# pennneutrinos/chroma

Hardware: AMD Instinct MI355X
Metric: photons/sec (propagate_hit) (higher is better)
Workload: dtype f32

## Files before the change

chroma_amd/csrc/chroma_hip.hip:

```cpp
#include <math.h>
#include <stdio.h>
#include <stdlib.h>
#include <string.h>
#include <algorithm>

#ifndef CHROMA_EXPERIMENTAL
#define CHROMA_EXPERIMENTAL 0
#endif
#ifndef CHROMA_HYBRID_RENDER
#define CHROMA_HYBRID_RENDER 1
#endif
#include "chroma_internal.h"
#include "propagate_device.h"

#include "kernel_propagate_fused.h"

#include "kernel_step_control.h"

#include "kernels_raycast_crosscheck.h"

#include "kernel_raycast_quad.h"

#include "kernel_raycast_pair.h"

// ... 123 lines not shown
        for (const Walk &w : WALKS)
            if (w.spill == b.kind) rays = std::max(rays, (size_t)ctx->waves[(int)w.cast] * w.rays_per_wave);
        HIP_TRY(hipSetDevice(ctx->device));
        HIP_TRY(ctx_malloc(ctx, (void **)b.buf, rays * b.depth * sizeof(uint2)));
    }
    return CHROMA_OK;
}

static unsigned cast_waves(const chroma_ctx *ctx, Cast cast, long long n)
{
    const long long per = WALKS[(int)cast].rays_per_wave;
    return (unsigned)std::min<long long>((n + per - 1) / per, ctx->waves[(int)cast]);
}

struct FusedLaunch { int first, nthreads; const uint32_t *in_q; uint32_t *out_q; int max_steps, use_weights, scatter_first; };
static int launch_propagate(const CallScope &scope, bool counting, chroma_geometry *geom, const PhotonView &pv, chroma_rng rng, const FusedLaunch &a)
{
    chroma_ctx *ctx = scope.ctx;
    const dim3 grid((unsigned)((a.nthreads + PROP_BLOCK - 1) / PROP_BLOCK)), block(PROP_BLOCK);
    with_bool(counting, [&](auto C) {
        hipLaunchKernelGGL((k_propagate<STACK_LDS, C>), grid, block, 0, ctx->stream, geom->view, pv, a.first, a.nthreads, a.in_q, a.out_q,
                           rng.seed, rng.photon_id_base, a.max_steps, a.use_weights, a.scatter_first, scope.state().d_counters);
    });
    HIP_TRY(hipGetLastError());
    return CHROMA_OK;
}

static int stats_read(const CallScope &scope, chroma_propagate_stats *stats)
{
    chroma_ctx *ctx = scope.ctx; CallState &cs = scope.state();
    DeviceCounters c;
    HIP_TRY(hipStreamSynchronize(ctx->stream));
    HIP_TRY(hipMemcpy(&c, cs.d_counters, sizeof c, hipMemcpyDeviceToHost));
    HIP_TRY(hipMemset(cs.d_counters, 0, sizeof c));
    stats->photon_steps += c.photon_steps;
    stats->nodes_visited += c.nodes_visited;
    stats->triangles_tested += c.triangles_tested;
    stats->stack_overflows += c.stack_overflows;
    stats->stack_spills += c.stack_spills;
    stats->packet_rays += c.packet_rays;
    stats->packet_nodes_visited += c.packet_nodes;
    stats->packet_triangles_tested += c.packet_tris;
    return CHROMA_OK;
}

enum { EV_STEP_BEGIN, EV_PACKET_BEGIN, EV_CAST_BEGIN, EV_CAST_END, EV_PHYSICS_END, EV_STEP_END, EV_PER_STEP };

struct chroma_tracks {
    struct Slab { float4 *rows; uint32_t count; };
    uint64_t nphotons = 0, nrows = 0;
    float4 *rows0 = nullptr;
    uint32_t *offsets = nullptr;
    std::vector<Slab> slabs;
};

static void tracks_release(chroma_ctx *ctx, chroma_tracks *tr)
{
    if (!tr) return;
    for (const chroma_tracks::Slab &s : tr->slabs) chroma_free(ctx, s.rows);
    chroma_free(ctx, tr->rows0);
    chroma_free(ctx, tr->offsets);
    delete tr;
}

namespace { struct PropagateCall; }
static int propagate_order(PropagateCall &call, uint32_t **d_order);

namespace {
struct PropagateCall {
    const CallScope &scope; CallState &cs;
    chroma_ctx *ctx; chroma_geometry *geom;
    CallPlan plan;
    PhotonView pv; chroma_rng rng; chroma_propagate_options opt;
    uint64_t nphotons; uint32_t ncopies;
    uint32_t *in_q, *out_q;
    float4 *work_in, *work_out;
    float4 *rays, *rays_next;
    float4 *final_rec;
    uint32_t final_epoch;
    HitsOut ho;
    bool finalize;
    chroma_propagate_stats acc;
    long long n_upper;
    bool finalized;
    chroma_tracks *tracks;

    hipEvent_t *events(int step) const { return opt.time_kernels ? cs.step_events.data() + EV_PER_STEP * step : nullptr; }

    int load_working()
    {
        const unsigned blocks = (unsigned)std::min<uint64_t>((nphotons + PHYS_BLOCK - 1) / PHYS_BLOCK, (uint64_t)ctx->physics_blocks);
        int rc = scope.clear_words(W_PACKET_USE, W_PACKET_END - W_PACKET_USE); if (rc) return rc;
        uint32_t *d_order = nullptr;
        rc = propagate_order(*this, &d_order); if (rc) return rc;
        hipLaunchKernelGGL(k_load_working, dim3(blocks), dim3(PHYS_BLOCK), 0, ctx->stream, geom->view, pv, in_q, work_in,
                           (uint64_t)nphotons, ncopies, (uint32_t)(nphotons / ncopies), plan.chain ? rays : nullptr,
                           plan.packet == 2 ? cs.d_words + W_PACKET_COHERENT : nullptr, (const uint32_t *)d_order, plan.cast == Cast::LITERAL ? 1 : 0);
        if (d_order) { chroma_free(ctx, d_order); acc.reordered += nphotons; }
#if CHROMA_EXPERIMENTAL
        if (plan.packet)
            hipLaunchKernelGGL(k_packet_decide, dim3(1), dim3(1), 0, ctx->stream, cs.d_words + W_PACKET_COHERENT, cs.d_words + W_PACKET_USE,
                               (uint64_t)nphotons, plan.packet);
#endif
        HIP_TRY(hipGetLastError());
        return CHROMA_OK;
    }

    void launch_step_begin(uint32_t first_n)
    {
        hipLaunchKernelGGL(k_step_begin, dim3(1), dim3(1), 0, ctx->stream, in_q, out_q, cs.d_step,
                           tracks ? 0u : opt.use_weights ? 0xFFFFFFFFu : (uint32_t)(PROP_BLOCK * 16 * 8), first_n);
    }

    void launch_physics(int scatter_first, int fixup)
    {
        StepState *st = cs.d_step;
        float4 *chained = plan.chain ? rays_next : nullptr;
        const bool plain = geom->view.plain_optics != 0;
        bool deal = false;
#if PHYS_DEAL
        deal = plain && !final_rec;
#endif
        const int pb = deal ? PHYS_DEAL_BLOCK : PHYS_BLOCK_OF(!plain);
        unsigned blocks = (unsigned)std::min<long long>((n_upper + pb - 1) / pb, std::max<long long>(1, (long long)ctx->physics_blocks * PHYS_BLOCK / pb));
        if (fixup == 1 && plain) blocks = std::max(std::min(blocks, 64u), blocks / 8);
        DeviceCounters *pc = plan.counting ? cs.d_counters : nullptr;
#if PHYS_DEAL
        if (deal) {
            hipLaunchKernelGGL(k_physics_deal, dim3(blocks), dim3(PHYS_DEAL_BLOCK), 0, ctx->stream, geom->view, pv, st, work_in, out_q, work_out,
                               cs.hit_triangle, cs.hit_distance, rng.seed, rng.photon_id_base, opt.use_weights, scatter_first,
                               cs.retry_list, fixup, pc, chained);
            return;
        }
#endif
        const int literal_rays = fixup == 2 ? 1 : 0;
        with_bool(!plain, [&](auto FULL) {
            hipLaunchKernelGGL((k_physics<FULL>), dim3(blocks), dim3(PHYS_BLOCK_OF(FULL)), 0, ctx->stream, geom->view, pv, st, work_in, out_q,
                               work_out, cs.hit_triangle, cs.hit_distance, rng.seed, rng.photon_id_base, opt.use_weights, scatter_first,
                               cs.retry_list, fixup, pc, chained, final_rec, final_epoch, literal_rays);
        });
    }

    int launch_split_step(int scatter_first, hipEvent_t *ev, uint32_t first_n, bool packet)
    {
        if (n_upper <= 0) return CHROMA_OK;
        StepState *st = cs.d_step;
        const Cast cast = plan.cast;
        const bool exact = cast == Cast::LITERAL || cast == Cast::LITERAL_LANE;
        const dim3 block(PROP_BLOCK);
        auto record = [&](int slot) { return ev ? hipEventRecord(ev[slot], ctx->stream) : hipSuccess; };
        const unsigned rblocks = (unsigned)std::min<long long>((n_upper + PROP_BLOCK - 1) / PROP_BLOCK, 8 * 256);
        auto retry = [&](auto C) {
            hipLaunchKernelGGL((k_raycast_retry<C>), dim3(rblocks), block, 0, ctx->stream, geom->view, rays, st, cs.hit_triangle,
                               cs.hit_distance, cs.retry_list, cs.d_counters);
        };
        launch_step_begin(first_n);
        HIP_TRY(record(EV_STEP_BEGIN));
        if (!plan.chain) {
            unsigned sblocks = (unsigned)std::min<long long>((n_upper + 255) / 256, (long long)ctx->physics_blocks * 4);
            hipLaunchKernelGGL(k_ray_setup, dim3(sblocks), dim3(256), 0, ctx->stream, geom->view, work_in, st, rays,
                               cs.hit_triangle, cs.hit_distance, cs.retry_list, &st->retry, cast == Cast::LITERAL ? 1 : 0);
        }
        HIP_TRY(record(EV_PACKET_BEGIN));
        const uint32_t *skip_quad = nullptr;
#if CHROMA_EXPERIMENTAL
        if (packet) {
            skip_quad = cs.d_words + W_PACKET_USE;
            const unsigned pwaves = (unsigned)std::min<long long>((n_upper + WAVE - 1) / WAVE, (long long)ctx->waves[(int)Cast::QUAD]);
            with_bool(plan.counting, [&](auto C) {
                hipLaunchKernelGGL((k_raycast_packet<C>), dim3(pwaves), block, 0, ctx->stream, geom->view, rays, st, cs.hit_triangle,
                                   cs.hit_distance, cs.retry_list, cs.d_counters, cs.d_words + W_PACKET_USE);
            });
        }
#else
        (void)packet;
#endif
        HIP_TRY(record(EV_CAST_BEGIN));
        const dim3 grid(cast_waves(ctx, cast, n_upper));
        const int chained = plan.chain ? 1 : 0;
        with_bool(plan.counting, [&](auto C) {
            switch (cast) {
            case Cast::PAIR:
                hipLaunchKernelGGL((k_raycast_pair<C>), grid, block, 0, ctx->stream, geom->view, rays, 0, st, cs.hit_triangle,
                                   cs.hit_distance, cs.retry_list, cs.coop_spill, cs.d_counters, ctx->coop_chunk);
                break;
            case Cast::QUAD:
                hipLaunchKernelGGL((k_raycast_quad<C>), grid, block, 0, ctx->stream, geom->view, rays, 0, st, cs.hit_triangle,
                                   cs.hit_distance, cs.retry_list, cs.coop_spill, cs.d_counters, ctx->coop_chunk, chained, skip_quad,
                                   ctx->claim_static);
                break;
            case Cast::COOP:
                hipLaunchKernelGGL((k_raycast_coop<C>), grid, block, 0, ctx->stream, geom->view, rays, 0, st, cs.hit_triangle,
                                   cs.hit_distance, cs.retry_list, cs.coop_spill, cs.d_counters, ctx->coop_chunk);
                break;
            case Cast::WIDE:
                hipLaunchKernelGGL((k_raycast_wide<C>), grid, block, 0, ctx->stream, geom->view, rays, 0, st, cs.hit_triangle,
                                   cs.hit_distance, cs.retry_list, cs.wide_spill, cs.d_counters, ctx->ray_chunk);
                break;
            case Cast::PERSISTENT:
                hipLaunchKernelGGL((k_raycast_persistent<C>), grid, block, 0, ctx->stream, geom->view, rays, 0, st, cs.hit_triangle,
                                   cs.hit_distance, cs.retry_list, cs.d_counters);
                break;
            case Cast::LITERAL:
                hipLaunchKernelGGL((k_raycast_literal<C>), grid, block, 0, ctx->stream, geom->view, rays, st, cs.hit_triangle,
                                   cs.hit_distance, cs.coop_spill, cs.d_counters, ctx->coop_chunk, chained, cs.retry_list,
                                   ctx->claim_static);
                retry(C);
                break;
            case Cast::LITERAL_LANE:
                hipLaunchKernelGGL((k_raycast_retry<C, true>), grid, block, 0, ctx->stream, geom->view, rays, st, cs.hit_triangle,
                                   cs.hit_distance, cs.retry_list, cs.d_counters);
                break;
            }
        });
        HIP_TRY(record(EV_CAST_END));
        launch_physics(scatter_first, exact ? 2 : 0);
        HIP_TRY(record(EV_PHYSICS_END));
        if (!exact) {
            with_bool(plan.counting, retry);
            launch_physics(scatter_first, 1);
        }
        HIP_TRY(record(EV_STEP_END));
        HIP_TRY(hipGetLastError());
        if (plan.chain) std::swap(rays, rays_next);
        return CHROMA_OK;
    }

    int launch_tail(int nsteps, int scatter_first, hipEvent_t *ev, uint32_t first_n, bool *done)
    {
        *done = false;
        const unsigned waves = cast_waves(ctx, Cast::COOP, n_upper);
        if ((long long)waves * 8 < n_upper) return CHROMA_OK;
        launch_step_begin(first_n);
        HitsOut beside; memset(&beside, 0, sizeof beside);
        uint32_t *words = nullptr;
        if (finalize) {
            beside = ho;
            words = cs.d_words;
            int rc = scope.clear_results(); if (rc) return rc;
            if (final_rec)
                hipLaunchKernelGGL(k_mark_tail, dim3(32), dim3(256), 0, ctx->stream, in_q, final_rec, photon_tail_stamp(final_epoch));
            HIP_TRY(hipEventRecord(cs.ev_fork, ctx->stream));
        }
        if (ev) HIP_TRY(hipEventRecord(ev[EV_STEP_BEGIN], ctx->stream));
        with_bool(plan.cast == Cast::LITERAL, [&](auto L) {
            with_bool(plan.counting, [&](auto C) {
                hipLaunchKernelGGL((k_tail_coop<C, L>), dim3(waves), dim3(PROP_BLOCK), 0, ctx->stream, geom->view, pv, cs.d_step, work_in,
                                   rng.seed, rng.photon_id_base, nsteps, opt.use_weights, scatter_first, cs.coop_spill, cs.d_counters, beside, words);
            });
        });
        if (ev) HIP_TRY(hipEventRecord(ev[EV_STEP_END], ctx->stream));
        if (finalize) {
            HIP_TRY(hipStreamWaitEvent(cs.aux_stream, cs.ev_fork, 0));
            launch_finalize(cs.aux_stream, photon_tail_stamp(final_epoch));
            HIP_TRY(hipEventRecord(cs.ev_join, cs.aux_stream));
            HIP_TRY(hipStreamWaitEvent(ctx->stream, cs.ev_join, 0));
            finalized = true;
        }
        HIP_TRY(hipGetLastError());
        *done = true;
        return CHROMA_OK;
    }

    void launch_finalize(hipStream_t stream, uint32_t tail_mark)
    {
        const unsigned blocks = (unsigned)((nphotons + COPY_ITEMS * 256 - 1) / (COPY_ITEMS * 256));
        hipLaunchKernelGGL(k_finalize_hits, dim3(blocks), dim3(256), 0, stream, geom->view, pv, (const float4 *)final_rec, final_epoch,
                           (uint64_t)nphotons, ho, cs.d_words, tail_mark);
    }

    int read_step_times(int steps, int tail_step)
    {
        for (int k = 0; k < steps; k++) {
            const hipEvent_t *ev = events(k);
            float ms = 0.f;
            HIP_TRY(hipEventElapsedTime(&ms, ev[EV_STEP_BEGIN], ev[EV_STEP_END]));
            acc.kernel_ms += ms;
            if (k == tail_step) continue;
            HIP_TRY(hipEventElapsedTime(&ms, ev[EV_CAST_BEGIN], ev[EV_CAST_END]));
            acc.raycast_ms += ms;
            acc.raycast_launches++;
            if (k == 0 && plan.packet) {
                HIP_TRY(hipEventElapsedTime(&ms, ev[EV_PACKET_BEGIN], ev[EV_CAST_BEGIN]));
                acc.packet_ms += ms;
                acc.packet_launches++;
            }
            HIP_TRY(hipEventElapsedTime(&ms, ev[EV_CAST_END], ev[EV_PHYSICS_END]));
            acc.physics_ms += ms;
            acc.physics_launches++;
        }
        return CHROMA_OK;
    }

    int run_device_steps()
    {
        const int max_steps = opt.max_steps;
        HIP_TRY(hipMemsetAsync(cs.d_step, 0, sizeof(StepState), ctx->stream));
        hipLaunchKernelGGL(k_set_word, dim3(1), dim3(1), 0, ctx->stream, in_q, 1u);
        hipLaunchKernelGGL(k_set_word, dim3(1), dim3(1), 0, ctx->stream, out_q, 1u);
        int rc = load_working(); if (rc) return rc;
        const int nev = opt.time_kernels ? EV_PER_STEP * max_steps : 0;
        while ((int)cs.step_events.size() < nev) { hipEvent_t e; HIP_TRY(hipEventCreate(&e)); cs.step_events.push_back(e); }
        const long long few = (long long)PROP_BLOCK * 16 * 8;
        int step = 0, next_check = 1, tail_step = -1;
        bool done = false;
        while (step < max_steps && !done) {
            const int scatter_first = step == 0 ? opt.scatter_first : 0;
            const uint32_t first_n = step == 0 ? (uint32_t)nphotons : 0u;
            if (plan.tail && n_upper < few) {
                rc = launch_tail(max_steps - step, scatter_first, events(step), first_n, &done); if (rc) return rc;
                if (done) { tail_step = step++; break; }
            }
            rc = launch_split_step(scatter_first, events(step), first_n, step == 0 && plan.packet != 0); if (rc) return rc;
            step++;
            std::swap(in_q, out_q);
            std::swap(work_in, work_out);
            if (step == next_check && step < max_steps) {
                rc = scope.read_survivors(in_q, &n_upper); if (rc) return rc;
                if (n_upper <= 0) done = true;
                next_check = (plan.tail_watch && n_upper < 16 * few) ? step + 1 : (step < 8) ? step * 2 : step + 8;
            }
        }
        if (!done) {
            unsigned blocks = (unsigned)std::min<long long>((n_upper + 255) / 256, 4096);
            hipLaunchKernelGGL(k_store_working, dim3(std::max(blocks, 1u)), dim3(256), 0, ctx->stream, geom->view, pv, in_q, work_in);
        }
        HIP_TRY(hipMemcpyAsync(cs.h_step, cs.d_step, sizeof(StepState), hipMemcpyDeviceToHost, ctx->stream));
        HIP_TRY(hipStreamSynchronize(ctx->stream));
        acc.launches += ((const StepState *)cs.h_step)->launches;
        return opt.time_kernels ? read_step_times(step, tail_step) : CHROMA_OK;
    }

    void store_working()
// ... 10 lines not shown
        hipLaunchKernelGGL(k_track_row0, dim3(tblocks), dim3(TRACK_BLOCK), 0, ctx->stream, pv, (uint64_t)nphotons, tr.rows0, tr.offsets,
                           (uint32_t)max_steps + 1u, max_steps >= 1 ? 2u : 1u);
        HIP_TRY(hipGetLastError());
        tr.nrows = nphotons;
        int step = 0;
        if (max_steps >= 1) {
            HIP_TRY(hipMemsetAsync(cs.d_step, 0, sizeof(StepState), ctx->stream));
            hipLaunchKernelGGL(k_set_word, dim3(1), dim3(1), 0, ctx->stream, in_q, 1u);
            hipLaunchKernelGGL(k_set_word, dim3(1), dim3(1), 0, ctx->stream, out_q, 1u);
            int rc = load_working(); if (rc) return rc;
            const int nev = opt.time_kernels ? EV_PER_STEP * max_steps : 0;
            while ((int)cs.step_events.size() < nev) { hipEvent_t e; HIP_TRY(hipEventCreate(&e)); cs.step_events.push_back(e); }
            rc = scope.read_survivors(in_q, &n_upper); if (rc) return rc;
            tr.nrows += nphotons - (uint64_t)n_upper;
            uint32_t *cursor = tr.offsets + nphotons + 1;
            while (step < max_steps && n_upper > 0) {
                const uint32_t n_in = (uint32_t)n_upper;
                chroma_tracks::Slab slab = {nullptr, n_in};
                if (step == 0) {
                    slab.rows = tr.slabs[0].rows;
                    tr.slabs.clear();
                    rc = CHROMA_OK;
                } else if (tr.nrows + n_in > max_rows)
                    rc = set_error(CHROMA_ERR_INVALID, "tracks: step %d would bring the call to %llu rows, more than the %llu of CHROMA_TRACKS_MAX_ROWS; %d steps were taken",
                                   step, (unsigned long long)(tr.nrows + n_in), (unsigned long long)max_rows, step);
                else
                    rc = chroma_malloc(ctx, (size_t)n_in * 4 * sizeof(float4), (void **)&slab.rows);
                if (rc) {
                    store_working();
                    hipStreamSynchronize(ctx->stream);
                    return rc;
                }
                tr.slabs.push_back(slab);
                HIP_TRY(hipMemsetAsync(cursor, 0, sizeof(uint32_t), ctx->stream));
                rc = launch_split_step(step == 0 ? opt.scatter_first : 0, events(step), step == 0 ? (uint32_t)nphotons : 0u, false);
                if (rc) return rc;
                const unsigned blocks = (unsigned)std::min<uint64_t>(((uint64_t)n_in + TRACK_BLOCK - 1) / TRACK_BLOCK, 4096);
                hipLaunchKernelGGL(k_track_step, dim3(blocks), dim3(TRACK_BLOCK), 0, ctx->stream, geom->view, pv, (const uint32_t *)in_q,
                                   (const uint32_t *)out_q, (const float4 *)work_out, slab.rows, n_in, cursor, tr.offsets, (uint32_t)step);
                HIP_TRY(hipGetLastError());
                tr.nrows += n_in;
                step++;
                std::swap(in_q, out_q);
                std::swap(work_in, work_out);
                rc = scope.read_survivors(in_q, &n_upper); if (rc) return rc;
            }
            if (n_upper > 0) store_working();
            HIP_TRY(hipMemcpyAsync(cs.h_step, cs.d_step, sizeof(StepState), hipMemcpyDeviceToHost, ctx->stream));
        }
        int rc = chroma_internal_exclusive_sum(ctx, tr.offsets, (uint32_t)nphotons + 1u); if (rc) return rc;
        HIP_TRY(hipStreamSynchronize(ctx->stream));
        uint32_t total = 0;
        HIP_TRY(hipMemcpy(&total, tr.offsets + nphotons, sizeof total, hipMemcpyDeviceToHost));
        if (total != tr.nrows)
            return set_error(CHROMA_ERR_INTERNAL, "tracks: %u rows recorded where the step counts give %llu", total, (unsigned long long)tr.nrows);
        if (max_steps >= 1) acc.launches += ((const StepState *)cs.h_step)->launches;
        return opt.time_kernels ? read_step_times(step, -1) : CHROMA_OK;
    }

    int run_fused()
    {
        hipLaunchKernelGGL(k_init_queue, dim3((unsigned)((nphotons + 255) / 256)), dim3(256), 0, ctx->stream, in_q,
                           (uint64_t)nphotons, ncopies, (uint32_t)(nphotons / ncopies));
        hipLaunchKernelGGL(k_set_word, dim3(1), dim3(1), 0, ctx->stream, out_q, 1u);
        HIP_TRY(hipGetLastError());
        const int max_steps = opt.max_steps;
        int scatter_first = opt.scatter_first;
        long long n = (long long)nphotons;
        int step = 0;
        while (step < max_steps) {
            const bool few = n < (long long)PROP_BLOCK * 16 * 8;
            int nsteps = (few || opt.use_weights) ? (max_steps - step) : 1;
            if (opt.time_kernels) HIP_TRY(hipEventRecord(cs.ev_start, ctx->stream));
            int rc = launch_propagate(scope, plan.counting, geom, pv, rng, {0, (int)n, in_q + 1, out_q, nsteps, opt.use_weights, scatter_first});
            if (rc) return rc;
            acc.launches++;
            if (opt.time_kernels) {
                HIP_TRY(hipEventRecord(cs.ev_stop, ctx->stream));
                HIP_TRY(hipEventSynchronize(cs.ev_stop));
                float ms = 0.f;
                HIP_TRY(hipEventElapsedTime(&ms, cs.ev_start, cs.ev_stop));
                acc.kernel_ms += ms;
            }
            step += nsteps;
            scatter_first = 0;
            if (step < max_steps) {
                std::swap(in_q, out_q);
                hipLaunchKernelGGL(k_set_word, dim3(1), dim3(1), 0, ctx->stream, out_q, 1u);
                rc = scope.read_survivors(in_q, &n); if (rc) return rc;
                if (n == 0) break;
            }
        }
        return CHROMA_OK;
    }

    int finish(chroma_hits_request *hr, chroma_propagate_stats *stats, int32_t *aborted)
    {
        int rc = CHROMA_OK;
        if (!finalize) {
            rc = scope.clear_words(W_ABORT); if (rc) return rc;
            const unsigned blocks = (unsigned)std::min<uint64_t>((nphotons + 255) / 256, 4096);
            hipLaunchKernelGGL(k_flags_or, dim3(blocks), dim3(256), 0, ctx->stream, pv.flags, (uint64_t)nphotons, CHROMA_NAN_ABORT,
                               cs.d_words + W_ABORT);
        } else if (!finalized) {
            rc = scope.clear_results(); if (rc) return rc;
            launch_finalize(ctx->stream, 0u);
        }
        HIP_TRY(hipGetLastError());
        rc = scope.read_results(); if (rc) return rc;
        if (hr) hr->nhits = scope.word(W_HIT_COUNT);
        if (aborted) *aborted = (scope.word(W_ABORT) & CHROMA_NAN_ABORT) ? 1 : 0;
        chroma_propagate_stats tmp; memset(&tmp, 0, sizeof tmp);
        chroma_propagate_stats *s = stats ? stats : &tmp;
        rc = stats_read(scope, s); if (rc) return rc;
        if (stats) {
            stats->launches += acc.launches;
            stats->kernel_ms += acc.kernel_ms;
            stats->raycast_ms += acc.raycast_ms;
            stats->raycast_launches += acc.raycast_launches;
            stats->physics_ms += acc.physics_ms;
            stats->physics_launches += acc.physics_launches;
            stats->packet_ms += acc.packet_ms;
            stats->packet_launches += acc.packet_launches;
            stats->reordered += acc.reordered;
        }
        if (s->stack_overflows) return set_error(CHROMA_ERR_STACK, "traversal stack overflowed for %llu rays", (unsigned long long)s->stack_overflows);
        return CHROMA_OK;
    }
};
}

int propagate_settings(const CallScope &scope)
{
    chroma_ctx *ctx = scope.ctx; CallState &cs = scope.state();
    hipDeviceProp_t prop;
    HIP_TRY(hipGetDeviceProperties(&prop, ctx->device));
    ctx->physics_blocks = prop.multiProcessorCount * 8;
    const char *walk = getenv("CHROMA_WALK");
    if (walk) cs.walk = CHROMA_WALK_QUAD;
    for (int w = 0; w < NWALKS; w++) {
        const Walk &row = WALKS[w];
        int per_cu = row.waves_per_cu;
        if (const char *e = getenv(row.waves_env)) per_cu = std::max(1, atoi(e));
        ctx->waves[(int)row.cast] = prop.multiProcessorCount * per_cu;
        if (walk && (!strcmp(walk, row.name) || (row.alias && !strcmp(walk, row.alias)))) cs.walk = w;
    }
#if CHROMA_EXPERIMENTAL
    if (const char *e = getenv("CHROMA_PACKET")) cs.packet_mode = !strcmp(e, "on") ? 1 : !strcmp(e, "auto") ? 2 : 0;
    if (const char *e = getenv("CHROMA_AUTOSORT")) cs.autosort_mode = !strcmp(e, "on") || !strcmp(e, "1") ? 1 : !strcmp(e, "off") || !strcmp(e, "0") ? 0 : 2;
#endif
    if (const char *e = getenv("CHROMA_RAY_CHUNK")) ctx->ray_chunk = std::max(64, atoi(e));
    if (const char *e = getenv("CHROMA_COOP_CHUNK")) ctx->coop_chunk = std::max(8, atoi(e));
    if (const char *e = getenv("CHROMA_CLAIM_STATIC")) { int big = 0, small = 0; if (sscanf(e, "%d:%d", &big, &small) < 2) small = big; ctx->claim_static = std::min(8, std::max(0, big)) | std::min(8, std::max(0, small)) << 4; }
    if (const char *e = getenv("CHROMA_TAIL"))
        cs.tail_mode = !strcmp(e, "fused") ? CHROMA_TAIL_FUSED : !strcmp(e, "split") ? CHROMA_TAIL_SPLIT : CHROMA_TAIL_COOP;
    return CHROMA_OK;
}

extern "C" {

int chroma_propagate_step(chroma_ctx *ctx, chroma_geometry *geom, int32_t first_photon, int32_t nthreads,
                          const uint32_t *d_input_queue, uint32_t *d_output_queue, chroma_rng rng,
                          const chroma_photon_arrays *photons, int32_t max_steps, int32_t use_weights,
                          int32_t scatter_first)
{
    if (!ctx || !geom) return set_error(CHROMA_ERR_INVALID, "bad argument");
    int rc = check_photons(photons, true);
    if (rc) return rc;
    if (first_photon < 0 || nthreads < 0) return set_error(CHROMA_ERR_INVALID, "negative photon range");
    if (nthreads == 0) return CHROMA_OK;
    if ((rc = check_stack(geom))) return rc;
    const CallScope scope(ctx);
    return launch_propagate(scope, scope.state().counting != 0, geom, to_view(photons), rng,
                            {first_photon, nthreads, d_input_queue, d_output_queue, max_steps, use_weights, scatter_first});
}

static int ensure_queues(const CallScope &scope, size_t n)
{
    chroma_ctx *ctx = scope.ctx; CallState &cs = scope.state();
    if (cs.queue_capacity >= n + 1) return CHROMA_OK;
    HIP_TRY(hipStreamSynchronize(ctx->stream));
    const auto buffers = queue_buffers(cs);
    for (const QueueBuffer &b : buffers) { if (*b.ptr) hipFree(*b.ptr); *b.ptr = nullptr; }
    cs.queue_capacity = 0;
    for (const QueueBuffer &b : buffers) HIP_TRY(ctx_malloc(ctx, b.ptr, (n + 1) * b.bytes));
    cs.queue_capacity = n + 1;
    return CHROMA_OK;
}

int chroma_distance_to_mesh(chroma_ctx *ctx, chroma_geometry *geom, int32_t nthreads, const float *d_origin,
                            const float *d_direction, float *d_distance, int32_t *d_triangle)
{
    return chroma_intersect_mesh(ctx, geom, nthreads, d_origin, d_direction, nullptr, d_distance, d_triangle);
}

int chroma_intersect_mesh(chroma_ctx *ctx, chroma_geometry *geom, int32_t nthreads, const float *d_origin,
                          const float *d_direction, const int32_t *d_last_hit, float *d_distance, int32_t *d_triangle)
{
    if (!ctx || !geom || !d_origin || !d_direction || !d_distance) return set_error(CHROMA_ERR_INVALID, "bad argument");
    if (nthreads <= 0) return CHROMA_OK;
    int rc = check_stack(geom); if (rc) return rc;
    const CallScope scope(ctx);
    CallState &cs = scope.state();
    CallPlan plan;
    rc = make_plan(cs, geom, -1, -1, -1, &plan); if (rc) return rc;
    if (!plan.isect_quad) {
        const dim3 grid((unsigned)((nthreads + PROP_BLOCK - 1) / PROP_BLOCK)), block(PROP_BLOCK);
        with_bool(plan.counting, [&](auto C) {
            hipLaunchKernelGGL((k_distance_to_mesh<STACK_LDS, C>), grid, block, 0, ctx->stream, geom->view, nthreads, d_origin, d_direction,
                               d_last_hit, d_distance, d_triangle, cs.d_counters);
        });
        HIP_TRY(hipGetLastError());
        return CHROMA_OK;
    }
    HIP_TRY(hipSetDevice(ctx->device));
    rc = ensure_queues(scope, (size_t)nthreads); if (rc) return rc;
    rc = ensure_spill(scope, SPILL_COOP); if (rc) return rc;
    StepState *st = cs.d_step;
    const unsigned blocks = (unsigned)((nthreads + 255) / 256);
    hipLaunchKernelGGL(k_step_set, dim3(1), dim3(1), 0, ctx->stream, st, (uint32_t)nthreads);
    hipLaunchKernelGGL(k_rays_from_arrays, dim3(blocks), dim3(256), 0, ctx->stream, geom->view, (int)nthreads, d_origin, d_direction,
                       d_last_hit, cs.rays, cs.hit_triangle, cs.hit_distance, cs.retry_list, st);
    const unsigned waves = cast_waves(ctx, Cast::QUAD, nthreads);
    with_bool(plan.counting, [&](auto C) {
        hipLaunchKernelGGL((k_raycast_quad<C>), dim3(waves), dim3(PROP_BLOCK), 0, ctx->stream, geom->view, cs.rays, 0, st,
                           cs.hit_triangle, cs.hit_distance, cs.retry_list, cs.coop_spill, cs.d_counters, ctx->coop_chunk, 0, nullptr, ctx->claim_static);
    });
    hipLaunchKernelGGL(k_distance_finish, dim3(blocks), dim3(256), 0, ctx->stream, geom->view, (int)nthreads, cs.rays, cs.hit_triangle,
                       cs.hit_distance, d_distance, d_triangle, cs.retry_list, st);
    with_bool(plan.counting, [&](auto C) {
        hipLaunchKernelGGL((k_distance_retry<C>), dim3(256), dim3(PROP_BLOCK), 0, ctx->stream, geom->view, cs.rays, st,
                           cs.retry_list, d_distance, d_triangle, cs.d_counters);
    });
    HIP_TRY(hipGetLastError());
    return CHROMA_OK;
}

int chroma_locate_materials(chroma_ctx *ctx, chroma_geometry *geom, int32_t n, const float *d_points, const float direction[3],
                            int32_t outside, int32_t *d_material, int32_t *d_triangle)
{
    if (!ctx || !geom || !d_points || !d_material) return set_error(CHROMA_ERR_INVALID, "bad argument");
    if (n < 0) return set_error(CHROMA_ERR_INVALID, "negative number of points");
    const float dx = direction ? direction[0] : 0.0f, dy = direction ? direction[1] : 0.0f, dz = direction ? direction[2] : 1.0f;
    const float len = sqrtf(dx * dx + dy * dy + dz * dz);
    if (!(len > 0.0f) || !isfinite(len)) return set_error(CHROMA_ERR_INVALID, "probe direction of no length");
    if (n == 0) return CHROMA_OK;
    int rc = check_stack(geom); if (rc) return rc;
    const CallScope scope(ctx);
    CallState &cs = scope.state();
    CallPlan plan;
    rc = make_plan(cs, geom, -1, -1, -1, &plan); if (rc) return rc;
    HIP_TRY(hipSetDevice(ctx->device));
    rc = ensure_queues(scope, (size_t)n); if (rc) return rc;
    int32_t *triangle = d_triangle ? d_triangle : cs.hit_triangle;
    const unsigned blocks = (unsigned)((n + 255) / 256);
    if (!plan.isect_quad) {
        with_bool(plan.counting, [&](auto C) {
            hipLaunchKernelGGL((k_locate_walk<STACK_LDS, C>), dim3((unsigned)((n + PROP_BLOCK - 1) / PROP_BLOCK)), dim3(PROP_BLOCK), 0, ctx->stream,
                               geom->view, (int)n, d_points, dx, dy, dz, triangle, cs.d_counters);
        });
    } else {
        rc = ensure_spill(scope, SPILL_COOP); if (rc) return rc;
        StepState *st = cs.d_step;
        hipLaunchKernelGGL(k_step_set, dim3(1), dim3(1), 0, ctx->stream, st, (uint32_t)n);
        hipLaunchKernelGGL(k_locate_rays, dim3(blocks), dim3(256), 0, ctx->stream, geom->view, (int)n, d_points, dx, dy, dz, cs.rays,
                           cs.hit_triangle, cs.hit_distance, cs.retry_list, st);
        const unsigned waves = cast_waves(ctx, Cast::QUAD, n);
        with_bool(plan.counting, [&](auto C) {
            hipLaunchKernelGGL((k_raycast_quad<C>), dim3(waves), dim3(PROP_BLOCK), 0, ctx->stream, geom->view, cs.rays, 0, st,
                               cs.hit_triangle, cs.hit_distance, cs.retry_list, cs.coop_spill, cs.d_counters, ctx->coop_chunk, 0, nullptr, ctx->claim_static);
        });
        hipLaunchKernelGGL(k_distance_finish, dim3(blocks), dim3(256), 0, ctx->stream, geom->view, (int)n, cs.rays, cs.hit_triangle,
                           cs.hit_distance, cs.hit_distance, triangle, cs.retry_list, st);
        with_bool(plan.counting, [&](auto C) {
            hipLaunchKernelGGL((k_distance_retry<C>), dim3(256), dim3(PROP_BLOCK), 0, ctx->stream, geom->view, cs.rays, st,
                               cs.retry_list, cs.hit_distance, triangle, cs.d_counters);
        });
    }
    hipLaunchKernelGGL(k_locate_material, dim3(blocks), dim3(256), 0, ctx->stream, geom->view, (int)n, triangle, dx, dy, dz, outside, d_material);
    HIP_TRY(hipGetLastError());
    return CHROMA_OK;
}

int chroma_propagate_stats_read(chroma_ctx *ctx, chroma_propagate_stats *stats)
{
    if (!ctx || !stats) return set_error(CHROMA_ERR_INVALID, "bad argument");
    const CallScope scope(ctx);
    return stats_read(scope, stats);
}

int chroma_set_counting(chroma_ctx *ctx, int32_t enabled)
{
    if (!ctx) return set_error(CHROMA_ERR_INVALID, "null ctx");
    CallScope(ctx).state().counting = enabled ? 1 : 0;
    return CHROMA_OK;
}

int chroma_set_walk(chroma_ctx *ctx, int32_t mode)
{
    if (!ctx) return set_error(CHROMA_ERR_INVALID, "null ctx");
    if (mode < 0 || mode >= NWALKS) return set_error(CHROMA_ERR_INVALID, "unknown walk mode %d", mode);
    CallScope(ctx).state().walk = mode;
    return CHROMA_OK;
}

int chroma_set_packet(chroma_ctx *ctx, int32_t mode)
// ... 318 lines not shown
```

chroma_amd/csrc/chroma_internal.h:

```cpp
#pragma once
#include <hip/hip_runtime.h>
#include <stdint.h>
#include <array>
#include <map>
#include <mutex>
#include <type_traits>
#include <unordered_map>
#include <vector>

#include <rccl/rccl.h>

#include "device_common.h"

#define CHROMA_LOCAL __attribute__((visibility("hidden")))

CHROMA_LOCAL int set_error(int code, const char *fmt, ...);

#define HIP_TRY(expr)                                                                          \
    do {                                                                                       \
        hipError_t e_ = (expr);                                                                \
        if (e_ != hipSuccess)                                                                  \
            return set_error((int)e_, "%s failed: %s (%s:%d)", #expr, hipGetErrorString(e_), __FILE__, __LINE__); \
    } while (0)

struct CallState {
    uint32_t *queue_a = nullptr, *queue_b = nullptr;
    size_t queue_capacity = 0;
    int32_t *hit_triangle = nullptr;
    float *hit_distance = nullptr;
    uint32_t *retry_list = nullptr;
    float4 *rays = nullptr;
    float4 *rays_b = nullptr;
    float4 *work_a = nullptr, *work_b = nullptr;
    float4 *final_rec = nullptr; size_t final_capacity = 0; uint32_t final_epoch = 0;
    DeviceCounters *d_counters = nullptr;
    uint32_t *d_words = nullptr;
    uint32_t *h_words = nullptr;
    StepState *d_step = nullptr;
    uint32_t *h_step = nullptr;
    std::vector<hipEvent_t> step_events;
    uint2 *wide_spill = nullptr;
    uint2 *coop_spill = nullptr;
    hipEvent_t ev_start = nullptr, ev_stop = nullptr, ev_mid = nullptr;
    hipStream_t aux_stream = nullptr;
    void *call_scratch = nullptr; size_t call_scratch_bytes = 0;
    hipEvent_t ev_fork = nullptr, ev_join = nullptr;
    int counting = 0;
    int tail_mode = CHROMA_TAIL_COOP;
    int autosort_mode = 0;
    int packet_mode = 0;
    int walk = CHROMA_WALK_QUAD;
};

struct chroma_ctx {
    int device;
    hipStream_t stream;
    int physics_blocks = 256 * 8;
    int waves[CHROMA_WALK_LITERAL_LANE + 1] = {};
    int ray_chunk = 256, coop_chunk = 64;
    int claim_static = 5 | 8 << 4;
    ncclComm_t comm = nullptr;
    int comm_nranks = 1, comm_rank = 0;
    uint32_t *gather_buf = nullptr;
    size_t gather_capacity = 0;
    struct PoolBlock { void *ptr; hipEvent_t ev; };
    std::mutex pool_mu;
    std::multimap<size_t, PoolBlock> pool;
    std::unordered_map<void *, size_t> live;
    std::vector<hipEvent_t> pool_events;
    size_t pool_bytes = 0, pool_limit = 0;
    uint64_t pool_hits = 0, pool_misses = 0;
    hipStream_t copy_stream = nullptr;
    std::mutex stage_mu;
    static constexpr int STAGE_N = 3;
    static constexpr size_t STAGE_BYTES = 64u << 20;
    void *stage[STAGE_N] = {nullptr, nullptr, nullptr};
    hipEvent_t stage_ev[STAGE_N] = {nullptr, nullptr, nullptr};
    std::mutex stage_down_mu;
    void *stage_down[STAGE_N] = {nullptr, nullptr, nullptr};
    hipEvent_t stage_down_ev[STAGE_N] = {nullptr, nullptr, nullptr};
private:
    friend class CallScope;
    std::mutex call_mu;
    CallState call_state;
};

struct chroma_geometry {
    chroma_ctx *ctx;
    GeoView view;
    std::vector<void *> allocations;
    void *d_vertices = nullptr, *d_triangles = nullptr, *d_material_codes = nullptr, *d_colors = nullptr;
    void *d_nodes_api = nullptr;
    size_t nvertices = 0, ntriangles = 0, nnodes = 0, nwide = 0, nrecords = 0;
    uint32_t stack_need = 0, wide_depth = 0, wide_stack_need = 0;
    size_t device_bytes = 0;
};

enum ScratchWord {
    W_HIT_COUNT = 0,
    W_SURVIVORS = 1,
    W_ABORT = 2,
    W_RESULT_END = 3,
    W_PACKET_USE = 4,
    W_PACKET_COHERENT = 5, W_PACKET_WAVES = 6, W_PACKET_END = 7,
    W_ORDER_PROBE = 8, W_ORDER_PROBE_END = 11,
    SCRATCH_WORDS = 16
};

class CallScope {
public:
    explicit CallScope(chroma_ctx *c) : ctx(c), lock_(c->call_mu) {}
    CallScope(const CallScope &) = delete;
    CallScope &operator=(const CallScope &) = delete;
    CallState &state() const { return ctx->call_state; }

    int clear_words(ScratchWord first, int count = 1) const
    {
        HIP_TRY(hipMemsetAsync(state().d_words + first, 0, count * sizeof(uint32_t), ctx->stream));
        return CHROMA_OK;
    }
    int clear_results() const { return clear_words(W_HIT_COUNT, W_RESULT_END - W_HIT_COUNT); }
    int read_words(ScratchWord first, int count = 1) const { return read_back(first, state().d_words + first, count); }
    int read_results() const { return read_words(W_HIT_COUNT, W_RESULT_END - W_HIT_COUNT); }
    uint32_t word(ScratchWord slot) const { return state().h_words[slot]; }
    int read_word(ScratchWord slot, uint32_t *out) const
    {
        const int rc = read_words(slot);
        *out = word(slot);
        return rc;
    }
    int read_survivors(const uint32_t *d_queue, long long *n) const
    {
        const int rc = read_back(W_SURVIVORS, d_queue, 1);
        *n = (long long)word(W_SURVIVORS) - 1;
        return rc;
    }

    chroma_ctx *const ctx;
private:
    int read_back(ScratchWord slot, const uint32_t *d_src, int count) const
    {
        HIP_TRY(hipMemcpyAsync(state().h_words + slot, d_src, count * sizeof(uint32_t), hipMemcpyDeviceToHost, ctx->stream));
        HIP_TRY(hipStreamSynchronize(ctx->stream));
        return CHROMA_OK;
    }
    std::lock_guard<std::mutex> lock_;
};

struct QueueBuffer { void **ptr; size_t bytes; };
static inline std::array<QueueBuffer, 9> queue_buffers(CallState &c)
{
    return {{{(void **)&c.queue_a, sizeof(uint32_t)}, {(void **)&c.queue_b, sizeof(uint32_t)},
             {(void **)&c.hit_triangle, sizeof(int32_t)}, {(void **)&c.hit_distance, sizeof(float)},
             {(void **)&c.retry_list, sizeof(uint32_t)}, {(void **)&c.rays, 4 * sizeof(float4)}, {(void **)&c.rays_b, 4 * sizeof(float4)},
             {(void **)&c.work_a, 4 * sizeof(float4)}, {(void **)&c.work_b, 4 * sizeof(float4)}}};
}

CHROMA_LOCAL hipError_t ctx_malloc(chroma_ctx *ctx, void **ptr, size_t bytes);

static int grow_call_scratch(const CallScope &scope, size_t need, bool *grew = nullptr)
{
    CallState &cs = scope.state();
    if (grew) *grew = false;
    if (cs.call_scratch_bytes >= need) return CHROMA_OK;
    HIP_TRY(hipStreamSynchronize(scope.ctx->stream));
    if (cs.call_scratch) { HIP_TRY(hipFree(cs.call_scratch)); cs.call_scratch = nullptr; cs.call_scratch_bytes = 0; }
    HIP_TRY(ctx_malloc(scope.ctx, &cs.call_scratch, need));
    cs.call_scratch_bytes = need;
    if (grew) *grew = true;
    return CHROMA_OK;
}

static inline size_t round256(size_t b) { return (b + 255) & ~(size_t)255; }
struct Carver {
    char *base = nullptr;
    size_t offset = 0;
    template <class T> T *take(size_t count)
    {
        T *p = base ? (T *)(base + offset) : nullptr;
        offset += round256(count * sizeof(T));
        return p;
    }
};
template <class Lay>
static int carve_call_scratch(const CallScope &scope, Lay &&lay, bool *grew = nullptr)
{
    Carver size;
    lay(size);
    int rc = grow_call_scratch(scope, size.offset, grew); if (rc) return rc;
    Carver block{(char *)scope.state().call_scratch};
    lay(block);
    return CHROMA_OK;
}

CHROMA_LOCAL int propagate_settings(const CallScope &scope);

extern "C" {
int chroma_internal_direction_order(chroma_ctx *ctx, const float *d_dir, uint32_t n, uint32_t *d_order);
int chroma_internal_sort_pairs(chroma_ctx *ctx, const uint32_t *d_keys, uint32_t *d_keys_out, const uint32_t *d_values,
                               uint32_t *d_values_out, uint32_t n, int end_bit);
int chroma_internal_exclusive_sum(chroma_ctx *ctx, uint32_t *d_counts, uint32_t n);
}
CHROMA_LOCAL int scan_workspace_bytes(size_t n, hipStream_t stream, size_t *bytes);
CHROMA_LOCAL int exclusive_sum(void *workspace, size_t bytes, uint32_t *d_in, uint32_t *d_out, size_t n, hipStream_t stream);
CHROMA_LOCAL int sort_pairs_workspace_bytes(size_t n, int end_bit, hipStream_t stream, size_t *bytes);
CHROMA_LOCAL int sort_pairs(void *workspace, size_t bytes, const uint64_t *d_keys, uint64_t *d_keys_out, const uint32_t *d_values,
                            uint32_t *d_values_out, size_t n, int end_bit, hipStream_t stream);

static PhotonView to_view(const chroma_photon_arrays *a)
{
    PhotonView v;
    v.pos = a->pos; v.dir = a->dir; v.pol = a->pol; v.wavelengths = a->wavelengths; v.t = a->t;
    v.flags = a->flags; v.last_hit_triangles = a->last_hit_triangles; v.weights = a->weights;
// ... 19 lines not shown
```

chroma_amd/csrc/kernel_raycast_literal.h:

```cpp
#pragma once

#ifndef LIT_STACK
#define LIT_STACK 32
#endif
#define LIT_STRIDE (LIT_STACK + 1)
#ifndef LIT_TRI_MIN
#define LIT_TRI_MIN 8
#endif
#ifndef LIT_TRI_END_HALF
#define LIT_TRI_END_HALF 1
#endif
#ifndef LIT_REFILL_MIN
#define LIT_REFILL_MIN 4
#endif
#ifndef LIT_WAVES_PER_EU
#define LIT_WAVES_PER_EU 8
#endif
#ifndef LIT_DIAG
#define LIT_DIAG 0
#endif
#define LIT_SPILL (2 * COOP_SPILL)

template <int K>
__device__ inline uint32_t quad_bcast_u32(uint32_t v)
// ... 79 lines not shown
                    noid = mk3(r3.x, r3.y, r3.z);
                    last_hit = __float_as_int(r0.w);
                    triangle_index = -1;
                    min_distance = -1.0f;
                    sp = 0;
                    cur = 0; end = 1;
                    has_ray = true;
                    active = true;
                    waiting = false;
                } else if (settle && j == 0) {
                    const int status = __float_as_int(r1.w);
                    hit_triangle[slot] = status;
                    hit_distance[slot] = 0.0f;
                    if (status == HIT_RETRY) retry_list[atomicAdd(&st->retry, 1u)] = (uint32_t)slot;
                }
            }
        }
        if (!__any(has_ray)) {
            if (exhausted && loc_next >= loc_end) break;
            continue;
        }

        more = !exhausted || loc_next < loc_end;
        const int stop_at = more ? max(0, (int)__popcll(__ballot(active && !waiting) & 0x1111111111111111ull) - (int)LIT_REFILL_MIN) : 0;
        const int tri_min = (more || !LIT_TRI_END_HALF) ? (int)LIT_TRI_MIN : max(1, min((int)LIT_TRI_MIN, ((int)__popcll(__ballot(has_ray) & 0x1111111111111111ull) + 1) / 2));
        do {
#if LIT_DIAG
            if (COUNT) { diag_iters++; diag_running += (unsigned)__popcll(__ballot(active && !waiting) & 0x1111111111111111ull); }
#endif
            __builtin_amdgcn_s_setprio(3);
            const bool pop = active && !waiting && cur >= end;
            if (__any(pop && sp > LIT_STACK)) {
                if (pop && sp > LIT_STACK) {
                    sp--;
                    const uint32_t w = spill[sp - LIT_STACK];
                    cur = w & ~CHROMA_NCHILD_MASK;
                    end = cur + (w >> CHROMA_CHILD_BITS);
                }
            } 
            if (pop && cur >= end) {
                if (sp == 0) {
                    active = false;
                } else {
                    sp--;
                    const uint32_t w = stack[sp];
                    cur = w & ~CHROMA_NCHILD_MASK;
                    end = cur + (w >> CHROMA_CHILD_BITS);
                }
            }
            if (active && !waiting) {
                const uint32_t idx = cur + j;
                const bool valid = idx < end;
                const uint4 nd = g.nodes[valid ? idx : end - 1u];
                __builtin_amdgcn_s_setprio(0);
                if (COUNT && j == 0 && end != 1u) cnt.nodes += min(4u, end - cur);
                cur += 4u;
                const float tmin = box_tmin_exact(nd, ws, wox, woy, woz, inv_dir, noid);
                const bool pass = valid && node_passes(tmin, min_distance);
                const bool leaf = (nd.w >> CHROMA_CHILD_BITS) == 0u;
                const bool is_tri = pass && leaf && (int)(nd.w & ~CHROMA_NCHILD_MASK) != last_hit;
                const bool is_inner = pass && !leaf;
                const uint32_t qm = quad_or_u32((is_inner ? (jbit << 4) : 0u) | (is_tri ? jbit : 0u));
                if ((qm & 0xFu) == 0u) {
                    const uint32_t mi = qm >> 4;
                    const int pos = sp + (int)__popc(mi & below);
                    if (is_inner) {
                        if (pos < LIT_STACK) stack[pos] = nd.w;
                        else if (pos < LIT_STACK + LIT_SPILL) { spill[pos - LIT_STACK] = nd.w; if (COUNT) cnt.spills++; }
                    }
                    sp += (int)__popc(mi);
                    if (sp > LIT_STACK + LIT_SPILL) { if (j == 0) cnt.overflows++; sp = LIT_STACK + LIT_SPILL; }
                } else {
                    waiting = true;
                    w_node = nd.w;
                    w_tmin = tmin;
                    w_qm = qm;
                }
            }
        } while ((int)__popcll(__ballot(waiting) & 0x1111111111111111ull) < tri_min &&
                 (int)__popcll(__ballot(active && !waiting) & 0x1111111111111111ull) > stop_at);
        __builtin_amdgcn_s_setprio(0);

        if (__any(waiting)) {
#if LIT_DIAG
            if (COUNT) { diag_passes++; diag_waiting += (unsigned)__popcll(__ballot(waiting) & 0x1111111111111111ull); }
#endif
            bool hit = false;
            float distance = 0.0f;
            if (waiting && (w_qm & jbit)) {
                hit = intersect_triangle_edges(origin, direction, g.tri_isect + 3 * (size_t)(w_node & ~CHROMA_NCHILD_MASK), distance);
            }
            const uint32_t hm = quad_or_u32(hit ? jbit : 0u);
            if (waiting) {
                const float t0 = quad_bcast_f32<0>(w_tmin), t1 = quad_bcast_f32<1>(w_tmin), t2 = quad_bcast_f32<2>(w_tmin), t3 = quad_bcast_f32<3>(w_tmin);
                const float d0 = quad_bcast_f32<0>(distance), d1 = quad_bcast_f32<1>(distance), d2 = quad_bcast_f32<2>(distance), d3 = quad_bcast_f32<3>(distance);
                float m = min_distance;
                uint32_t win = 4u, acc = 0u, ntested = 0u;
#define LIT_REPLAY(K, TK, DK)                                                                                          \
                if ((w_qm & (0x11u << K)) && node_passes(TK, m)) {                                                     \
                    if (w_qm & (1u << K)) {                                                                            \
                        ntested++;                                                                                     \
                        if ((hm & (1u << K)) && (m < 0.0f || DK < m)) { m = DK; win = K; }               \
                    } else {                                                                                           \
                        acc |= 1u << K;                                                                                \
                    }                                                                                                  \
                }
                LIT_REPLAY(0, t0, d0) LIT_REPLAY(1, t1, d1) LIT_REPLAY(2, t2, d2) LIT_REPLAY(3, t3, d3)
#undef LIT_REPLAY
                if (COUNT && j == 0) cnt.tris += ntested;
                const uint32_t wchild = quad_max_u32(j == win ? (w_node & ~CHROMA_NCHILD_MASK) + 1u : 0u);
                if (win != 4u) { triangle_index = (int)wchild - 1; min_distance = m; }
                if (acc) {
                    const int pos = sp + (int)__popc(acc & below);
                    if (acc & jbit) {
                        if (pos < LIT_STACK) stack[pos] = w_node;
                        else if (pos < LIT_STACK + LIT_SPILL) { spill[pos - LIT_STACK] = w_node; if (COUNT) cnt.spills++; }
                    }
                    sp += (int)__popc(acc);
                    if (sp > LIT_STACK + LIT_SPILL) { if (j == 0) cnt.overflows++; sp = LIT_STACK + LIT_SPILL; }
                }
            }
            waiting = false;
            __builtin_amdgcn_wave_barrier();
        }

        if (has_ray && !active) {
            if (j == 0) {
                hit_triangle[slot] = triangle_index;
                hit_distance[slot] = min_distance;
            }
            has_ray = false;
        }
    }

    const unsigned long long ov = wave_sum_u64(cnt.overflows);
    if (COUNT) {
        const unsigned long long nd = wave_sum_u64(cnt.nodes), tr = wave_sum_u64(cnt.tris), sx = wave_sum_u64(cnt.spills);
        if (lane == 0) {
            atomicAdd(&counters->nodes_visited, nd);
            atomicAdd(&counters->triangles_tested, tr);
            if (sx) atomicAdd(&counters->stack_spills, sx);
        }
    }
    if (lane == 0 && ov) atomicAdd(&counters->stack_overflows, ov);
#if LIT_DIAG
    if (COUNT && lane == 0) {
        atomicAdd(&counters->packet_nodes, (unsigned long long)diag_iters);
        atomicAdd(&counters->packet_rays, (unsigned long long)diag_running);
        atomicAdd(&counters->packet_tris, ((unsigned long long)diag_waiting << 32) | diag_passes);
    }
#endif
}

template <bool COUNT>
__device__ inline int literal_cast_group8(const GeoView &g, v3 origin, v3 direction, int last_hit, bool on, float &min_distance,
                                          uint32_t *stack, uint32_t *spill, unsigned j8, LaneCounters &cnt)
{
    const unsigned j = j8 & 3u;
    const uint32_t jbit = 1u << j, below = jbit - 1u;
    const float ws = g.world_scale, wox = g.world_origin[0], woy = g.world_origin[1], woz = g.world_origin[2];
    int triangle_index = -1;
    min_distance = -1.0f;
    v3 noid = mk3(0.f, 0.f, 0.f), inv_dir = mk3(0.f, 0.f, 1.f);
    bool active = false;
    if (on) {
        noid = (-origin) / direction;
        inv_dir = 1.0f / direction;
        const bool moderate = cm_fabsf(inv_dir.x) < 1e30f && cm_fabsf(inv_dir.y) < 1e30f && cm_fabsf(inv_dir.z) < 1e30f &&
                              cm_fabsf(noid.x) < 1e30f && cm_fabsf(noid.y) < 1e30f && cm_fabsf(noid.z) < 1e30f;
        if (!moderate) triangle_index = HIT_RETRY; else active = true;
    }
    uint32_t cur = 0, end = 1;
    int sp = 0;
    while (__any(active)) {
        if (active && cur >= end) {
            if (sp == 0) {
                active = false;
            } else {
                sp--;
                const uint32_t w = (sp < LIT_STACK) ? stack[sp] : spill[sp - LIT_STACK];
                cur = w & ~CHROMA_NCHILD_MASK;
                end = cur + (w >> CHROMA_CHILD_BITS);
            }
        }
        if (active) {
            const uint32_t idx = cur + j;
            const bool valid = idx < end;
            const uint4 nd = g.nodes[valid ? idx : end - 1u];
            if (COUNT && j8 == 0 && end != 1u) cnt.nodes += min(4u, end - cur);
            cur += 4u;
            const float tmin = box_tmin_exact(nd, ws, wox, woy, woz, inv_dir, noid);
            const bool pass = valid && node_passes(tmin, min_distance);
            const bool leaf = (nd.w >> CHROMA_CHILD_BITS) == 0u;
            const bool is_tri = pass && leaf && (int)(nd.w & ~CHROMA_NCHILD_MASK) != last_hit;
            const bool is_inner = pass && !leaf;
            const uint32_t qm = quad_or_u32((is_inner ? (jbit << 4) : 0u) | (is_tri ? jbit : 0u));
            uint32_t acc = qm >> 4;
            if (qm & 0xFu) {
                bool hit = false;
                float distance = 0.0f;
                if (is_tri) {
                    hit = intersect_triangle_edges(origin, direction, g.tri_isect + 3 * (size_t)(nd.w & ~CHROMA_NCHILD_MASK), distance);
                }
                const uint32_t hm = quad_or_u32(hit ? jbit : 0u);
                const float t0 = quad_bcast_f32<0>(tmin), t1 = quad_bcast_f32<1>(tmin), t2 = quad_bcast_f32<2>(tmin), t3 = quad_bcast_f32<3>(tmin);
                const float d0 = quad_bcast_f32<0>(distance), d1 = quad_bcast_f32<1>(distance), d2 = quad_bcast_f32<2>(distance), d3 = quad_bcast_f32<3>(distance);
                float m = min_distance;
                uint32_t win = 4u, ntested = 0u;
                acc = 0u;
#define LIT_REPLAY(K, TK, DK)                                                                                          \
                if ((qm & (0x11u << K)) && node_passes(TK, m)) {                                                       \
                    if (qm & (1u << K)) {                                                                              \
                        ntested++;                                                                                     \
                        if ((hm & (1u << K)) && (m < 0.0f || DK < m)) { m = DK; win = K; }               \
                    } else {                                                                                           \
                        acc |= 1u << K;                                                                                \
                    }                                                                                                  \
                }
                LIT_REPLAY(0, t0, d0) LIT_REPLAY(1, t1, d1) LIT_REPLAY(2, t2, d2) LIT_REPLAY(3, t3, d3)
#undef LIT_REPLAY
                if (COUNT && j8 == 0) cnt.tris += ntested;
                const uint32_t wchild = quad_max_u32(j == win ? (nd.w & ~CHROMA_NCHILD_MASK) + 1u : 0u);
                if (win != 4u) { triangle_index = (int)wchild - 1; min_distance = m; }
            }
            if (acc) {
                const int pos = sp + (int)__popc(acc & below);
                if ((acc & jbit) && j8 < 4u) {
                    if (pos < LIT_STACK) stack[pos] = nd.w;
                    else if (pos < LIT_STACK + LIT_SPILL) { spill[pos - LIT_STACK] = nd.w; if (COUNT) cnt.spills++; }
                }
                sp += (int)__popc(acc);
                if (sp > LIT_STACK + LIT_SPILL) { if (j8 == 0) cnt.overflows++; sp = LIT_STACK + LIT_SPILL; }
            }
            __builtin_amdgcn_wave_barrier();
        }
    }
    return triangle_index;
}
```

chroma_amd/csrc/kernel_raycast_retry.h:

```cpp
#pragma once

template <bool COUNT, bool ALL = false>
__global__ __launch_bounds__(PROP_BLOCK) void
k_raycast_retry(GeoView g, const float4 *rays, const StepState *st,
                int32_t *hit_triangle, float *hit_distance, const uint32_t *retry_list, DeviceCounters *counters)
{
    const int nretry = ALL ? (int)st->n : (int)st->retry;
    __shared__ uint32_t s_lds[TRAV_LDS_WORDS(STACK_LDS, PROP_BLOCK)];
    if (nretry == 0) return;
    LaneCounters cnt = {0, 0, 0, 0};
    const int stride = gridDim.x * PROP_BLOCK;
    for (int k0 = blockIdx.x * PROP_BLOCK; k0 < nretry; k0 += stride) {
        const int k = k0 + (int)threadIdx.x;
        bool walk = false;
        int slot = 0, last_hit = -1;
        v3 position = mk3(0.f, 0.f, 0.f), direction = mk3(0.f, 0.f, 1.f);
        if (k < nretry) {
            slot = ALL ? k : (int)retry_list[k];
            const float4 *r = rays + 4 * (size_t)slot;
            const float4 r0 = r[0], r1 = r[1];
            position = mk3(r0.x, r0.y, r0.z); direction = mk3(r1.x, r1.y, r1.z);
            last_hit = __float_as_int(r0.w);
        }
        if (ALL) {
            walk = k < nretry && __float_as_int(rays[4 * (size_t)slot + 1].w) != HIT_NAN;
        } else if (k < nretry) {
            const int rec = hit_triangle[slot];
            walk = true;
            if (rec >= 0) {
                const float4 *t = g.tri + TRI_STRIDE * (size_t)rec;
                walk = !record_hit_is_exactly_regular(g, t[0], t[1], t[2], position, direction, hit_distance[slot]);
            }
        }
        float dist;
        int found = intersect_mesh_dev<STACK_LDS, PROP_BLOCK, COUNT>(g, position, direction, dist, last_hit, s_lds + threadIdx.x, cnt, walk);
        if (walk) {
            hit_triangle[slot] = found;
            hit_distance[slot] = dist;
        }
    }
    flush_counters<COUNT, FLUSH_STEPS | FLUSH_OVERFLOWS>(cnt, counters, lane_id());
}
```

Measured before the change: 898.8 million.

## Walk retry rays with four-lane cooperative literal traversal

The retry kernel now compacts rays that need a re-walk and traverses each one with a quad of four lanes, using a generalized literal_cast_group templated on group size and stack depth, instead of one lane per ray. This targets divergence and long serial traversals in the retry pass. Rays whose inverse direction or origin term is not finite still fall back to the per-lane walk. A separate option can turn off counting in the non-exact cast kernels, and both behaviors are controlled by environment variables, with quad retry on by default.

```diff
diff --git a/chroma_amd/csrc/chroma_hip.hip b/chroma_amd/csrc/chroma_hip.hip
--- a/chroma_amd/csrc/chroma_hip.hip
+++ b/chroma_amd/csrc/chroma_hip.hip
@@ -299,7 +299,7 @@
         const unsigned rblocks = (unsigned)std::min<long long>((n_upper + PROP_BLOCK - 1) / PROP_BLOCK, 8 * 256);
         auto retry = [&](auto C) {
             hipLaunchKernelGGL((k_raycast_retry<C>), dim3(rblocks), block, 0, ctx->stream, geom->view, rays, st, cs.hit_triangle,
-                               cs.hit_distance, cs.retry_list, cs.d_counters);
+                               cs.hit_distance, cs.retry_list, cs.d_counters, ctx->retry_lanes == 4 ? 1 : 0);
         };
         launch_step_begin(first_n);
         HIP_TRY(record(EV_STEP_BEGIN));
@@ -325,7 +325,7 @@
         HIP_TRY(record(EV_CAST_BEGIN));
         const dim3 grid(cast_waves(ctx, cast, n_upper));
         const int chained = plan.chain ? 1 : 0;
-        with_bool(plan.counting, [&](auto C) {
+        with_bool(plan.counting && !(ctx->count_rewalk_only && !exact), [&](auto C) {
             switch (cast) {
             case Cast::PAIR:
                 hipLaunchKernelGGL((k_raycast_pair<C>), grid, block, 0, ctx->stream, geom->view, rays, 0, st, cs.hit_triangle,
@@ -642,6 +642,8 @@
     if (const char *e = getenv("CHROMA_RAY_CHUNK")) ctx->ray_chunk = std::max(64, atoi(e));
     if (const char *e = getenv("CHROMA_COOP_CHUNK")) ctx->coop_chunk = std::max(8, atoi(e));
     if (const char *e = getenv("CHROMA_CLAIM_STATIC")) { int big = 0, small = 0; if (sscanf(e, "%d:%d", &big, &small) < 2) small = big; ctx->claim_static = std::min(8, std::max(0, big)) | std::min(8, std::max(0, small)) << 4; }
+    if (const char *e = getenv("CHROMA_RETRY_LANES")) ctx->retry_lanes = atoi(e) == 1 ? 1 : 4;
+    if (const char *e = getenv("CHROMA_COUNT_REWALK_ONLY")) ctx->count_rewalk_only = atoi(e) != 0;
     if (const char *e = getenv("CHROMA_TAIL"))
         cs.tail_mode = !strcmp(e, "fused") ? CHROMA_TAIL_FUSED : !strcmp(e, "split") ? CHROMA_TAIL_SPLIT : CHROMA_TAIL_COOP;
     return CHROMA_OK;
diff --git a/chroma_amd/csrc/chroma_internal.h b/chroma_amd/csrc/chroma_internal.h
--- a/chroma_amd/csrc/chroma_internal.h
+++ b/chroma_amd/csrc/chroma_internal.h
@@ -59,6 +59,8 @@
     int waves[CHROMA_WALK_LITERAL_LANE + 1] = {};
     int ray_chunk = 256, coop_chunk = 64;
     int claim_static = 5 | 8 << 4;
+    int retry_lanes = 4;
+    int count_rewalk_only = 0;
     ncclComm_t comm = nullptr;
     int comm_nranks = 1, comm_rank = 0;
     uint32_t *gather_buf = nullptr;
diff --git a/chroma_amd/csrc/kernel_raycast_literal.h b/chroma_amd/csrc/kernel_raycast_literal.h
--- a/chroma_amd/csrc/kernel_raycast_literal.h
+++ b/chroma_amd/csrc/kernel_raycast_literal.h
@@ -255,10 +255,11 @@
 #endif
 }
 
-template <bool COUNT>
-__device__ inline int literal_cast_group8(const GeoView &g, v3 origin, v3 direction, int last_hit, bool on, float &min_distance,
-                                          uint32_t *stack, uint32_t *spill, unsigned j8, LaneCounters &cnt)
-{
+template <bool COUNT, unsigned GROUP, int STACK_N, int SPILL_N>
+__device__ inline int literal_cast_group(const GeoView &g, v3 origin, v3 direction, int last_hit, bool on, float &min_distance,
+                                         uint32_t *stack, uint32_t *spill, unsigned j8, LaneCounters &cnt)
+{
+    static_assert(GROUP == 4u || GROUP == 8u, "one quad or two");
     const unsigned j = j8 & 3u;
     const uint32_t jbit = 1u << j, below = jbit - 1u;
     const float ws = g.world_scale, wox = g.world_origin[0], woy = g.world_origin[1], woz = g.world_origin[2];
@@ -281,7 +282,7 @@
                 active = false;
             } else {
                 sp--;
-                const uint32_t w = (sp < LIT_STACK) ? stack[sp] : spill[sp - LIT_STACK];
+                const uint32_t w = (SPILL_N == 0 || sp < STACK_N) ? stack[sp] : spill[sp - STACK_N];
                 cur = w & ~CHROMA_NCHILD_MASK;
                 end = cur + (w >> CHROMA_CHILD_BITS);
             }
@@ -328,15 +329,21 @@
             }
             if (acc) {
                 const int pos = sp + (int)__popc(acc & below);
-                if ((acc & jbit) && j8 < 4u) {
-                    if (pos < LIT_STACK) stack[pos] = nd.w;
-                    else if (pos < LIT_STACK + LIT_SPILL) { spill[pos - LIT_STACK] = nd.w; if (COUNT) cnt.spills++; }
+                if ((acc & jbit) && (GROUP == 4u || j8 < 4u)) {
+                    if (pos < STACK_N) stack[pos] = nd.w;
+                    else if (SPILL_N > 0 && pos < STACK_N + SPILL_N) { spill[pos - STACK_N] = nd.w; if (COUNT) cnt.spills++; }
                 }
                 sp += (int)__popc(acc);
-                if (sp > LIT_STACK + LIT_SPILL) { if (j8 == 0) cnt.overflows++; sp = LIT_STACK + LIT_SPILL; }
+                if (sp > STACK_N + SPILL_N) { if (j8 == 0) cnt.overflows++; sp = STACK_N + SPILL_N; }
             }
             __builtin_amdgcn_wave_barrier();
         }
     }
     return triangle_index;
 }
+template <bool COUNT>
+__device__ inline int literal_cast_group8(const GeoView &g, v3 origin, v3 direction, int last_hit, bool on, float &min_distance,
+                                          uint32_t *stack, uint32_t *spill, unsigned j8, LaneCounters &cnt)
+{
+    return literal_cast_group<COUNT, 8u, LIT_STACK, LIT_SPILL>(g, origin, direction, last_hit, on, min_distance, stack, spill, j8, cnt);
+}
diff --git a/chroma_amd/csrc/kernel_raycast_retry.h b/chroma_amd/csrc/kernel_raycast_retry.h
--- a/chroma_amd/csrc/kernel_raycast_retry.h
+++ b/chroma_amd/csrc/kernel_raycast_retry.h
@@ -1,15 +1,23 @@
 #pragma once
+
+#define RETRY_QSTACK (STACK_LDS + STACK_SCRATCH)
+#define RETRY_QSTRIDE (RETRY_QSTACK + 1)
 
 template <bool COUNT, bool ALL = false>
 __global__ __launch_bounds__(PROP_BLOCK) void
 k_raycast_retry(GeoView g, const float4 *rays, const StepState *st,
-                int32_t *hit_triangle, float *hit_distance, const uint32_t *retry_list, DeviceCounters *counters)
+                int32_t *hit_triangle, float *hit_distance, const uint32_t *retry_list, DeviceCounters *counters, int quad_lanes = 0)
 {
     const int nretry = ALL ? (int)st->n : (int)st->retry;
-    __shared__ uint32_t s_lds[TRAV_LDS_WORDS(STACK_LDS, PROP_BLOCK)];
+    constexpr int LANE_WORDS = TRAV_LDS_WORDS(STACK_LDS, PROP_BLOCK);
+    constexpr int QUAD_WORDS = 16 * RETRY_QSTRIDE + WAVE;
+    constexpr bool QUAD = !ALL;
+    static_assert(PROP_BLOCK == WAVE, "one wave per workgroup");
+    __shared__ uint32_t s_lds[(QUAD && QUAD_WORDS > LANE_WORDS) ? QUAD_WORDS : LANE_WORDS];
     if (nretry == 0) return;
     LaneCounters cnt = {0, 0, 0, 0};
     const int stride = gridDim.x * PROP_BLOCK;
+    const unsigned lane = lane_id();
     for (int k0 = blockIdx.x * PROP_BLOCK; k0 < nretry; k0 += stride) {
         const int k = k0 + (int)threadIdx.x;
         bool walk = false;
@@ -32,6 +40,38 @@
                 walk = !record_hit_is_exactly_regular(g, t[0], t[1], t[2], position, direction, hit_distance[slot]);
             }
         }
+        if (QUAD && quad_lanes) {
+            bool quad = false;
+            if (walk) {
+                const v3 noid = (-position) / direction, inv_dir = 1.0f / direction;
+                quad = cm_fabsf(inv_dir.x) < 1e30f && cm_fabsf(inv_dir.y) < 1e30f && cm_fabsf(inv_dir.z) < 1e30f &&
+                       cm_fabsf(noid.x) < 1e30f && cm_fabsf(noid.y) < 1e30f && cm_fabsf(noid.z) < 1e30f;
+            }
+            const unsigned long long qmask = __ballot(quad);
+            if (qmask) {
+                const int nq = __popcll(qmask);
+                const unsigned j = lane & 3u, grp = lane >> 2;
+                uint32_t *src_lane = s_lds + 16 * RETRY_QSTRIDE;
+                if (quad) src_lane[__popcll(qmask & ((1ull << lane) - 1ull))] = lane;
+                __builtin_amdgcn_wave_barrier();
+                for (int q0 = 0; q0 < nq; q0 += 16) {
+                    const bool on = q0 + (int)grp < nq;
+                    const int src = on ? (int)src_lane[q0 + (int)grp] : (int)lane;
+                    const v3 o = mk3(__shfl(position.x, src), __shfl(position.y, src), __shfl(position.z, src));
+                    const v3 d = mk3(__shfl(direction.x, src), __shfl(direction.y, src), __shfl(direction.z, src));
+                    const int lh = __shfl(last_hit, src), qslot = __shfl(slot, src);
+                    float qdist;
+                    const int found = literal_cast_group<COUNT, 4u, RETRY_QSTACK, 0>(g, o, d, lh, on, qdist, s_lds + grp * RETRY_QSTRIDE,
+                                                                                    nullptr, j, cnt);
+                    if (on && j == 0) {
+                        hit_triangle[qslot] = found;
+                        hit_distance[qslot] = qdist;
+                    }
+                }
+                __builtin_amdgcn_wave_barrier();
+            }
+            walk = walk && !quad;
+        }
         float dist;
         int found = intersect_mesh_dev<STACK_LDS, PROP_BLOCK, COUNT>(g, position, direction, dist, last_hit, s_lds + threadIdx.x, cnt, walk);
         if (walk) {
```

After: 903.0 million (median of 6 runs). About the same (+0.5%).
